# wuwuz/Pacmann

Measured on AMD Instinct MI355X. Metric: private queries/sec + PIR-scan HBM GB/s, SIFT1M d=128 at 1/2/4/8 GPUs, higher is better.
Workload: dtype u64

## Files before the change

### pacmann_amd/csrc/pm_aes.h

```cpp
#pragma once
#include <hip/hip_runtime.h>
#include <stdint.h>

namespace pm {

struct AesTables {
  uint8_t sbox[256];
  uint32_t te0[256];
  constexpr AesTables() : sbox(), te0() {
    for (int x = 0; x < 256; ++x) {
      uint8_t inv = 0;
      if (x) {
        uint8_t r = 1, b = (uint8_t)x;
        int e = 254;
        while (e) {
          if (e & 1) r = gmul(r, b);
          b = gmul(b, b);
          e >>= 1;
        }
        inv = r;
      }
      uint8_t s = inv ^ rotl(inv, 1) ^ rotl(inv, 2) ^ rotl(inv, 3) ^ rotl(inv, 4) ^ 0x63;
      sbox[x] = s;
      uint32_t s2 = gmul(s, 2), s3 = gmul(s, 3);
      te0[x] = s2 | ((uint32_t)s << 8) | ((uint32_t)s << 16) | (s3 << 24);
    }
  }
  static constexpr uint8_t gmul(uint8_t a, uint8_t b) {
    uint8_t p = 0;
    for (int i = 0; i < 8; ++i) {
      if (b & 1) p ^= a;
      bool hi = a & 0x80;
      a = (uint8_t)(a << 1);
      if (hi) a ^= 0x1b;
      b >>= 1;
    }
    return p;
  }
  static constexpr uint8_t rotl(uint8_t v, int n) { return (uint8_t)((v << n) | (v >> (8 - n))); }
};

constexpr int kTeLdsWords = 256 * 64;

static constexpr AesTables kAesTablesHost{};
static __device__ const AesTables g_aes = kAesTablesHost;

__device__ __forceinline__ uint32_t rotl32(uint32_t x, int n) { return (x << n) | (x >> (32 - n)); }
__device__ __forceinline__ uint32_t aes_x3(uint32_t a, uint32_t b, uint32_t c) {
  return __builtin_amdgcn_bitop3_b32(a, b, c, 0x96);
}

__device__ __forceinline__ void aes_lds_init(uint32_t* te, const uint32_t* __restrict__ g_te0) {
  for (int i = threadIdx.x; i < kTeLdsWords; i += blockDim.x) {
    const uint32_t t = g_te0[(i >> 6) & 255];
    te[i] = (i & 32) ? rotl32(t, 16) : t;
  }
}


struct AesLane {
  const uint32_t* te;
  uint32_t lane;
  uint32_t lane2;
  __device__ AesLane(const uint32_t* t, uint32_t tid) : te(t), lane((tid & 31u) << 2), lane2(((tid & 31u) << 2) | 0x80u) {}
  template <int K> __device__ __forceinline__ uint32_t Tk(uint32_t s) const {
    const uint32_t a = __builtin_amdgcn_perm(s, lane, 0x0c0c0000u | ((4u + K) << 8));
    return *reinterpret_cast<const uint32_t*>(reinterpret_cast<const char*>(te) + a);
  }
  template <int K> __device__ __forceinline__ uint32_t T2k(uint32_t s) const {
    const uint32_t a = __builtin_amdgcn_perm(s, lane2, 0x0c0c0000u | ((4u + K) << 8));
    return *reinterpret_cast<const uint32_t*>(reinterpret_cast<const char*>(te) + a);
  }
  template <int K> __device__ __forceinline__ uint32_t Sk(uint32_t s) const { return (Tk<K>(s) >> 8) & 0xffu; }
  __device__ __forceinline__ uint32_t col(uint32_t a, uint32_t b, uint32_t c, uint32_t d, uint32_t k) const {
    return __builtin_amdgcn_bitop3_b32(__builtin_amdgcn_bitop3_b32(Tk<0>(a), T2k<2>(c), k, 0x96),
                                       rotl32(Tk<1>(b) ^ T2k<3>(d), 8), 0u, 0x96);
  }
};

template <int R0 = 1, int R1 = 10>
__device__ __forceinline__ void aes_rounds(const AesLane& A, const uint32_t* __restrict__ rk,
                                           uint32_t& s0, uint32_t& s1, uint32_t& s2, uint32_t& s3) {
#pragma unroll
  for (int r = R0; r < R1; ++r) {
    uint32_t t0 = A.col(s0, s1, s2, s3, rk[4 * r + 0]);
    uint32_t t1 = A.col(s1, s2, s3, s0, rk[4 * r + 1]);
    uint32_t t2 = A.col(s2, s3, s0, s1, rk[4 * r + 2]);
    uint32_t t3 = A.col(s3, s0, s1, s2, rk[4 * r + 3]);
    s0 = t0; s1 = t1; s2 = t2; s3 = t3;
  }
}

__device__ __forceinline__ uint64_t prf64(const AesLane& A, const uint32_t* __restrict__ rk,
                                          uint64_t tag, uint64_t x) {
  const uint64_t b = (tag << 35) + x;
  const uint32_t w0 = (uint32_t)b, w1 = (uint32_t)(b >> 32);
  uint32_t s0 = w0 ^ rk[0], s1 = w1 ^ rk[1], s2 = rk[2], s3 = rk[3];
  aes_rounds(A, rk, s0, s1, s2, s3);
  uint32_t c0 = (A.Sk<0>(s0) | (A.Sk<1>(s1) << 8) | (A.Sk<2>(s2) << 16) | (A.Sk<3>(s3) << 24)) ^ rk[40];
  uint32_t c1 = (A.Sk<0>(s1) | (A.Sk<1>(s2) << 8) | (A.Sk<2>(s3) << 16) | (A.Sk<3>(s0) << 24)) ^ rk[41];
  return ((uint64_t)(c1 ^ w1) << 32) | (uint64_t)(c0 ^ w0);
}

__device__ __forceinline__ uint32_t prf_lo32(const AesLane& A, const uint32_t* __restrict__ rk,
                                             uint64_t tag, uint64_t x) {
  const uint64_t b = (tag << 35) + x;
  const uint32_t w0 = (uint32_t)b, w1 = (uint32_t)(b >> 32);
  uint32_t s0 = w0 ^ rk[0], s1 = w1 ^ rk[1], s2 = rk[2], s3 = rk[3];
  aes_rounds(A, rk, s0, s1, s2, s3);
  uint32_t c0 = (A.Sk<0>(s0) | (A.Sk<1>(s1) << 8) | (A.Sk<2>(s2) << 16) | (A.Sk<3>(s3) << 24)) ^ rk[40];
  return c0 ^ w0;
}

struct R1Uniform { uint32_t u0, u1, u2, u3; };
__device__ __forceinline__ R1Uniform r1_uniform(const AesLane& A, const uint32_t* __restrict__ rk, uint32_t x) {
  const uint32_t s0 = x ^ rk[0], s2 = rk[2], s3 = rk[3];
  return R1Uniform{A.Tk<0>(s0) ^ A.T2k<2>(s2) ^ rotl32(A.T2k<3>(s3), 8) ^ rk[4],
                   A.T2k<2>(s3) ^ rotl32(A.Tk<1>(s2) ^ A.T2k<3>(s0), 8) ^ rk[5],
                   A.Tk<0>(s2) ^ A.T2k<2>(s0) ^ rotl32(A.Tk<1>(s3), 8) ^ rk[6],
                   A.Tk<0>(s3) ^ rotl32(A.Tk<1>(s0) ^ A.T2k<3>(s2), 8) ^ rk[7]};
}
struct R1Lane { uint32_t v0, v1, v2, v3; };
__device__ __forceinline__ R1Lane r1_lane(const AesLane& A, const uint32_t* __restrict__ rk, uint64_t tag) {
  const uint32_t s1 = (uint32_t)(tag << 3) ^ rk[1];
  return R1Lane{rotl32(A.Tk<1>(s1), 8), A.Tk<0>(s1), rotl32(A.T2k<3>(s1), 8), A.T2k<2>(s1)};
}
__device__ __forceinline__ uint32_t prf_lo32_split(const AesLane& A, const uint32_t* __restrict__ rk,
                                                   const R1Uniform& u, const R1Lane& v, uint32_t x) {
  uint32_t s0 = u.u0 ^ v.v0, s1 = u.u1 ^ v.v1, s2 = u.u2 ^ v.v2, s3 = u.u3 ^ v.v3;
  aes_rounds<2>(A, rk, s0, s1, s2, s3);
  const uint32_t c0 = (A.Sk<0>(s0) | (A.Sk<1>(s1) << 8) | (A.Sk<2>(s2) << 16) | (A.Sk<3>(s3) << 24)) ^ rk[40];
  return c0 ^ x;
}

__device__ __forceinline__ uint32_t prf_lo16_split(const AesLane& A, const uint32_t* __restrict__ rk,
                                                   const R1Uniform& u, const R1Lane& v, uint32_t x) {
  uint32_t s0 = u.u0 ^ v.v0, s1 = u.u1 ^ v.v1, s2 = u.u2 ^ v.v2, s3 = u.u3 ^ v.v3;
  aes_rounds<2, 9>(A, rk, s0, s1, s2, s3);
  const uint32_t t0 = A.col(s0, s1, s2, s3, rk[36]);
  const uint32_t t1 = A.col(s1, s2, s3, s0, rk[37]);
  return ((A.Sk<0>(t0) | (A.Sk<1>(t1) << 8)) ^ rk[40] ^ x) & 0xffffu;
}
struct R2Hint { uint32_t k0, k1, k2, k3; };
__device__ __forceinline__ R2Hint r2_hint(const AesLane& A, const uint32_t* __restrict__ rk, const R1Uniform& u,
                                          const R1Lane& v) {
  const uint32_t s1 = u.u1 ^ v.v1, s2 = u.u2 ^ v.v2, s3 = u.u3 ^ v.v3;
  return R2Hint{A.T2k<2>(s2) ^ rk[8] ^ rotl32(A.Tk<1>(s1) ^ A.T2k<3>(s3), 8),
                A.Tk<0>(s1) ^ A.T2k<2>(s3) ^ rk[9] ^ rotl32(A.Tk<1>(s2), 8),
                A.Tk<0>(s2) ^ rk[10] ^ rotl32(A.Tk<1>(s3) ^ A.T2k<3>(s1), 8),
                A.Tk<0>(s3) ^ A.T2k<2>(s1) ^ rk[11] ^ rotl32(A.T2k<3>(s2), 8)};
}
__device__ __forceinline__ uint32_t prf_lo16_r2(const AesLane& A, const uint32_t* __restrict__ rk, uint32_t u0,
                                                const R1Lane& v, const R2Hint& k, uint32_t x) {
  const uint32_t s = u0 ^ v.v0;
  uint32_t s0 = A.Tk<0>(s) ^ k.k0, s1 = rotl32(A.T2k<3>(s), 8) ^ k.k1;
  uint32_t s2 = A.T2k<2>(s) ^ k.k2, s3 = rotl32(A.Tk<1>(s), 8) ^ k.k3;
  aes_rounds<3, 9>(A, rk, s0, s1, s2, s3);
  const uint32_t t0 = A.col(s0, s1, s2, s3, rk[36]);
  const uint32_t t1 = A.col(s1, s2, s3, s0, rk[37]);
  return ((A.Sk<0>(t0) | (A.Sk<1>(t1) << 8)) ^ rk[40] ^ x) & 0xffffu;
}
}
```

### pacmann_amd/csrc/pm_kernels.hip

```cpp
#include <atomic>
#include "pm_aes.h"
#include "pm_aes_bs.h"
#include "pm_internal.h"

namespace pm {
#ifndef PM_PREP_NT
#define PM_PREP_NT 0
#endif


__device__ __forceinline__ uint32_t xor3(uint32_t a, uint32_t b, uint32_t c) {
  return __builtin_amdgcn_bitop3_b32(a, b, c, 0x96);
}
__device__ __forceinline__ uint4 xor4(uint4 a, uint4 b) {
  return make_uint4(a.x ^ b.x, a.y ^ b.y, a.z ^ b.z, a.w ^ b.w);
}

#ifndef PM_OFFS_CHUNKS
#define PM_OFFS_CHUNKS 8
#endif
constexpr int kOffsChunksPerBlock = PM_OFFS_CHUNKS;
constexpr int kOffsBlock = 1024;

#ifndef PM_OFFS_TILES
#define PM_OFFS_TILES 1
#endif
constexpr int kOffsTiles = PM_OFFS_TILES;
__global__ void __launch_bounds__(kOffsBlock, 1) k_prep_offsets(const PmPart* __restrict__ parts) {
  __shared__ uint32_t te[kTeLdsWords];
  __shared__ R1Uniform r1u[kOffsTiles][kOffsChunksPerBlock];
  const PmPart& P = parts[blockIdx.z];
  const uint32_t H = P.H, SS = P.SS;
  const uint32_t cb = blockIdx.y * kOffsChunksPerBlock * kOffsTiles;
  if (blockIdx.x * kOffsBlock >= H || cb >= SS) return;
  aes_lds_init(te, g_aes.te0);
  __syncthreads();
  const AesLane A(te, threadIdx.x);
  const uint32_t cend = min(SS, cb + kOffsChunksPerBlock * kOffsTiles);
  if (threadIdx.x < cend - cb)
    r1u[threadIdx.x / kOffsChunksPerBlock][threadIdx.x % kOffsChunksPerBlock] = r1_uniform(A, P.rk, cb + threadIdx.x);
  __syncthreads();
  const uint32_t h = blockIdx.x * kOffsBlock + threadIdx.x;
  if (h >= H) return;
  const uint32_t mask = P.CS - 1;
  const uint32_t own = h >= P.PH ? (h - P.PH) / P.Qpc : 0xffffffffu;
  uint16_t* o = P.tab;
  const R1Lane r1v = r1_lane(A, P.rk, h);
  const bool r2 = SS <= 256;
  const R2Hint r2k = r2 ? r2_hint(A, P.rk, r1u[0][0], r1v) : R2Hint{0, 0, 0, 0};
  static_assert(kOffsChunksPerBlock == 8, "one 16-B tabT tile of 8 chunks per thread");
  for (int tl = 0; tl < kOffsTiles; ++tl) {
    const uint32_t c0 = cb + tl * kOffsChunksPerBlock;
    if (c0 >= SS) break;
    const uint32_t c1 = min(SS, c0 + kOffsChunksPerBlock);
    uint16_t tile[8];
#pragma unroll
    for (int j = 0; j < 8; ++j) tile[j] = kSkip;
    auto put = [&](uint32_t c, uint32_t prf) {
      uint16_t v = (uint16_t)(prf & mask);
      v = (c == own) ? kSkip : v;
      if (o) o[(uint64_t)c * H + h] = v;
      tile[c - c0] = v;
      if (h < P.PH) P.cur[cur_index(P.PH, P.curk, c, h)] = v;
    };
    for (uint32_t c = c0; c < c1; ++c)
      put(c, r2 ? prf_lo16_r2(A, P.rk, r1u[tl][c - c0].u0, r1v, r2k, c) : prf_lo16_split(A, P.rk, r1u[tl][c - c0], r1v, c));
    uint4 t4;
    t4.x = tile[0] | ((uint32_t)tile[1] << 16); t4.y = tile[2] | ((uint32_t)tile[3] << 16);
    t4.z = tile[4] | ((uint32_t)tile[5] << 16); t4.w = tile[6] | ((uint32_t)tile[7] << 16);
    if (PM_PREP_NT) {
      typedef uint32_t u32x4 __attribute__((ext_vector_type(4)));
      __builtin_nontemporal_store(u32x4{t4.x, t4.y, t4.z, t4.w}, reinterpret_cast<u32x4*>(P.tabT + tabT_index(H, h, c0)));
    } else {
      *reinterpret_cast<uint4*>(P.tabT + tabT_index(H, h, c0)) = t4;
    }
  }
}

constexpr int kBsThreads = 256;
#ifndef PM_BS_WAVES
#define PM_BS_WAVES 2
#endif
__global__ void __launch_bounds__(kBsThreads, PM_BS_WAVES) k_prep_offsets_bs(const PmPart* __restrict__ parts) {
  __shared__ uint32_t bs_te0[256];
  __shared__ uint32_t bs_kx[32];
  __shared__ uint32_t bs_wv[32][4];
  __shared__ __attribute__((aligned(16))) uint32_t bs_wp[128];
  __shared__ __attribute__((aligned(16))) uint32_t bs_stash[16 * kBsThreads];
  const PmPart& P = parts[blockIdx.y];
  const uint32_t H = P.H, SS = P.SS, PH = P.PH;
  const uint32_t nm = (H + 31) / 32, ng = (SS + 7) / 8;
  if (blockIdx.x * kBsThreads >= nm * ng) return;
  bs_te0[threadIdx.x] = g_aes.te0[threadIdx.x];
  __syncthreads();
  bs_setup_a(bs_te0, P.rk, bs_kx, bs_wv);
  __syncthreads();
  bs_setup_b(bs_wv, bs_wp);
  __syncthreads();
  const uint32_t task = blockIdx.x * kBsThreads + threadIdx.x;
  if (task >= nm * ng) return;
  const uint32_t m = task % nm, g = task / nm, h0 = 32 * m;
  const uint32_t nb = P.log2CS, Qpc = P.Qpc;
  const uint32_t keep = nb >= 16 ? 0xffffu : (1u << nb) - 1u;
  auto lowmask = [](int n) { return n <= 0 ? 0u : n >= 32 ? ~0u : (1u << n) - 1u; };
  uint4* stash = reinterpret_cast<uint4*>(bs_stash) + threadIdx.x;
#pragma unroll 1
  for (uint32_t q = 0; q < 8; ++q) {
    const uint32_t cc = 8 * g + q, c = cc & ~1u;
    uint32_t T[32];
    if (c < SS) {
      uint32_t o[16];
      bs_prf16(bs_te0, P.rk, bs_kx, bs_wp, m, cc, o);
      const int lo = (int)(PH + cc * Qpc) - (int)h0, hi = lo + (int)Qpc;
      const uint32_t own = lowmask(hi) & ~lowmask(lo);
#pragma unroll
      for (int b = 0; b < 16; ++b) o[b] = (((keep >> b) & 1u) ? o[b] : 0u) | own;
      if ((q & 1) == 0) {
#pragma unroll
        for (int i = 0; i < 4; ++i) stash[i * kBsThreads] = make_uint4(o[4 * i], o[4 * i + 1], o[4 * i + 2], o[4 * i + 3]);
        continue;
      }
#pragma unroll
      for (int i = 0; i < 4; ++i) {
        const uint4 v = stash[i * kBsThreads];
        T[4 * i] = v.x; T[4 * i + 1] = v.y; T[4 * i + 2] = v.z; T[4 * i + 3] = v.w;
      }
#pragma unroll
      for (int b = 0; b < 16; ++b) T[16 + b] = o[b];
      bs_transpose32(T);
    } else {
      if ((q & 1) == 0) continue;
#pragma unroll
      for (int j = 0; j < 32; ++j) T[j] = 0xffffffffu;
    }
    uint32_t* tt = reinterpret_cast<uint32_t*>(P.tabT + tabT_index(H, h0, c));
    if (h0 + 32 <= H) {
#pragma unroll
      for (int j = 0; j < 32; ++j) tt[4 * j] = T[j];
    } else {
#pragma unroll
      for (int j = 0; j < 32; ++j)
        if (h0 + j < H) tt[4 * j] = T[j];
    }
    if (c >= SS) continue;
#pragma unroll
    for (int jb = 0; jb < 4; ++jb) {
      const uint32_t hb = h0 + 8 * jb;
      uint4 wlo, whi;
      wlo.x = __builtin_amdgcn_perm(T[8 * jb + 1], T[8 * jb + 0], 0x05040100u);
      wlo.y = __builtin_amdgcn_perm(T[8 * jb + 3], T[8 * jb + 2], 0x05040100u);
      wlo.z = __builtin_amdgcn_perm(T[8 * jb + 5], T[8 * jb + 4], 0x05040100u);
      wlo.w = __builtin_amdgcn_perm(T[8 * jb + 7], T[8 * jb + 6], 0x05040100u);
      whi.x = __builtin_amdgcn_perm(T[8 * jb + 1], T[8 * jb + 0], 0x07060302u);
      whi.y = __builtin_amdgcn_perm(T[8 * jb + 3], T[8 * jb + 2], 0x07060302u);
      whi.z = __builtin_amdgcn_perm(T[8 * jb + 5], T[8 * jb + 4], 0x07060302u);
      whi.w = __builtin_amdgcn_perm(T[8 * jb + 7], T[8 * jb + 6], 0x07060302u);
      if (hb < PH) {
        *reinterpret_cast<uint4*>(P.cur + cur_index(PH, P.curk, c, hb)) = wlo;
        *reinterpret_cast<uint4*>(P.cur + cur_index(PH, P.curk, c + 1, hb)) = whi;
      }
      if (P.tab && hb < H) {
        *reinterpret_cast<uint4*>(P.tab + (uint64_t)c * H + hb) = wlo;
        *reinterpret_cast<uint4*>(P.tab + (uint64_t)(c + 1) * H + hb) = whi;
      }
    }
  }
}

#ifndef PM_FOLD_NT
#define PM_FOLD_NT 1
#endif
template <int W>
__global__ void __launch_bounds__(kBlock) k_prep_fold(const PmPart* __restrict__ parts,
                                                      const uint64_t* __restrict__ db, uint32_t E) {
  const PmPart& P = parts[blockIdx.y];
  const uint32_t EX = E & ~3u, NSEG = EX / W;
  const uint64_t e = (uint64_t)blockIdx.x * kBlock + threadIdx.x;
  const uint32_t H = P.H;
  if (NSEG == 0) {
    if (e < (uint64_t)H * E) P.parity[e] = 0;
    return;
  }
  const uint32_t h = (uint32_t)(e / NSEG), seg = (uint32_t)(e % NSEG);
  if (h >= H) return;
  const uint64_t* base = db + (P.row0 * E) + (uint64_t)seg * W;
  const uint32_t CS = P.CS, SS = P.SS;
  const uint64_t N = P.N;
  uint64_t a0 = 0, a1 = 0;
  uint32_t c = 0;
  for (; c + 4 <= SS; c += 4) {
    const uint64_t t4 = *reinterpret_cast<const uint64_t*>(P.tabT + tabT_index(H, h, c));
    uint16_t v[4];
#pragma unroll
    for (int u = 0; u < 4; ++u) v[u] = (uint16_t)(t4 >> (16 * u));
#pragma unroll
    for (int u = 0; u < 4; ++u) {
      const uint64_t r = (uint64_t)(c + u) * CS + v[u];
      if (v[u] != kSkip && r < N) {
        const uint64_t* p = base + r * E;
        if (W == 2) {
          typedef uint32_t u32x4 __attribute__((ext_vector_type(4)));
          const u32x4 x = PM_FOLD_NT ? __builtin_nontemporal_load(reinterpret_cast<const u32x4*>(p))
                                     : *reinterpret_cast<const u32x4*>(p);
          a0 ^= ((uint64_t)x.y << 32) | x.x;
          a1 ^= ((uint64_t)x.w << 32) | x.z;
        } else {
          a0 ^= PM_FOLD_NT ? __builtin_nontemporal_load(p) : *p;
        }
      }
    }
  }
  for (; c < SS; ++c) {
    uint16_t v = P.tabT[tabT_index(H, h, c)];
    const uint64_t r = (uint64_t)c * CS + v;
    if (v != kSkip && r < N) {
      const uint64_t* p = base + r * E;
      a0 ^= p[0];
      if (W == 2) a1 ^= p[1];
    }
  }
  uint64_t* dst = P.parity + (uint64_t)h * E + (uint64_t)seg * W;
  dst[0] = a0;
  if (W == 2) dst[1] = a1;
  if (seg == 0)
    for (uint32_t w = EX; w < E; ++w) P.parity[(uint64_t)h * E + w] = 0;
}

constexpr int kFoldThreads = 1024, kFoldHPT = 7;
// ... 565 lines not shown
          if (r >= P.N) continue;
          const uint64_t* p = base + r * rw + (uint64_t)seg * W;
          if (W == 2) {
            const uint4 x = *reinterpret_cast<const uint4*>(p);
            x0[u] = ((uint64_t)x.y << 32) | x.x;
            x1[u] = ((uint64_t)x.w << 32) | x.z;
          } else {
            x0[u] = *p;
          }
        }
#pragma unroll
        for (uint32_t u = 0; u < kSrvFlight; ++u) { a0 ^= x0[u]; a1 ^= x1[u]; }
      }
    }
    red[threadIdx.x * 2] = a0;
    red[threadIdx.x * 2 + 1] = a1;
    __syncthreads();
    if (threadIdx.x < nseg) {
      uint64_t x0 = 0, x1 = 0;
      for (uint32_t k = 0; k < nsl; ++k) {
        x0 ^= red[(k * nseg + threadIdx.x) * 2];
        x1 ^= red[(k * nseg + threadIdx.x) * 2 + 1];
      }
      if (PK && seg < cseg) {
        const uint32_t v[4] = {(uint32_t)x0, (uint32_t)(x0 >> 32), (uint32_t)x1, (uint32_t)(x1 >> 32)};
#pragma unroll
        for (uint32_t k = 0; k < 4; ++k)
          out[4 * seg + k] = ((uint64_t)(v[k] & 0xffff0000u) << 32) | (uint64_t)(uint32_t)(v[k] << 16);
      } else if (PK) {
        out[4 * cseg + 2 * (seg - cseg)] = x0;
        out[4 * cseg + 2 * (seg - cseg) + 1] = x1;
      } else {
        out[(uint64_t)seg * W] = x0;
        if (W == 2) out[(uint64_t)seg * W + 1] = x1;
      }
    }
    __syncthreads();
  }
  for (uint32_t w = (E & ~3u) + threadIdx.x; w < E; w += kBlock) out[w] = 0;
}

__global__ void __launch_bounds__(kBlock) k_l2_rows(const float* __restrict__ rows,
                                                    uint64_t stride, uint64_t nrows,
                                                    const uint32_t* __restrict__ ids,
                                                    const float* __restrict__ q, uint32_t dim,
                                                    float* __restrict__ out, uint64_t seglen) {
  const uint64_t g = ((uint64_t)blockIdx.x * kBlock + threadIdx.x) >> 3;
  const uint32_t k = threadIdx.x & 7;
  const bool live = g < nrows;
  const float* r = rows + (live ? (ids ? (uint64_t)ids[g] : g) : 0) * stride;
  if (seglen && live) q += (g / seglen) * dim;
  const uint32_t dimS = dim & ~7u;
  float acc = 0.0f;
  if (live)
    for (uint32_t t = k; t < dimS; t += 8) {
      const float d = __fsub_rn(r[t], q[t]);
      acc = __fadd_rn(acc, __fmul_rn(d, d));
    }
  acc = __fadd_rn(acc, __shfl_xor(acc, 1));
  acc = __fadd_rn(acc, __shfl_xor(acc, 2));
  acc = __fadd_rn(acc, __shfl_xor(acc, 4));
  if (live && k == 0) {
    float d = dimS ? acc : 0.0f;
    for (uint32_t i = dimS; i < dim; ++i) {
      const float t = __fsub_rn(r[i], q[i]);
      d = __fadd_rn(d, __fmul_rn(t, t));
    }
    out[g] = d;
  }
}

__global__ void __launch_bounds__(kBlock) k_ip_rows(const uint32_t* __restrict__ rows, uint64_t nrows,
                                                    const uint32_t* __restrict__ q, uint32_t dim,
                                                    uint32_t* __restrict__ per_row,
                                                    uint32_t* __restrict__ sum) {
  const uint64_t g = ((uint64_t)blockIdx.x * kBlock + threadIdx.x) >> 4;
  const uint32_t l = threadIdx.x & 15;
  uint32_t acc = 0;
  if (g < nrows) {
    const uint32_t* r = rows + g * dim;
    for (uint32_t j = l; j < dim; j += 16) acc += r[j] * q[j];
  }
#pragma unroll
  for (int m = 1; m < 16; m <<= 1) acc += __shfl_xor(acc, m);
  if (g < nrows && l == 0 && per_row) per_row[g] = acc;
  uint32_t w = (l == 0 && g < nrows) ? acc : 0;
#pragma unroll
  for (int m = 16; m < 64; m <<= 1) w += __shfl_xor(w, m);
  if ((threadIdx.x & 63) == 0) atomicAdd(sum, w);
}

__global__ void __launch_bounds__(kBlock) k_ip_scan(const uint4* __restrict__ rows, uint64_t n4,
                                                    const uint32_t* __restrict__ q, uint32_t dim,
                                                    uint32_t* __restrict__ sum) {
  __shared__ uint32_t qs[4096];
  for (uint32_t j = threadIdx.x; j < dim; j += kBlock) qs[j] = q[j];
  __syncthreads();
  uint32_t acc = 0;
  const uint64_t stride = (uint64_t)gridDim.x * kBlock;
  const uint32_t dim4 = dim / 4;
  typedef unsigned int u32x4 __attribute__((ext_vector_type(4)));
  const u32x4* r4 = reinterpret_cast<const u32x4*>(rows);
  uint64_t f = (uint64_t)blockIdx.x * kBlock + threadIdx.x;
  if (stride % dim4 == 0) {
    const uint32_t j = (uint32_t)(f % dim4) * 4;
    const uint32_t q0 = qs[j], q1 = qs[j + 1], q2 = qs[j + 2], q3 = qs[j + 3];
    constexpr int kU = 8;
    for (; f + (kU - 1) * stride < n4; f += kU * stride) {
      u32x4 t[kU];
#pragma unroll
      for (int u = 0; u < kU; ++u) t[u] = __builtin_nontemporal_load(r4 + f + u * stride);
#pragma unroll
      for (int u = 0; u < kU; ++u) acc += t[u].x * q0 + t[u].y * q1 + t[u].z * q2 + t[u].w * q3;
    }
    for (; f < n4; f += stride) {
      const u32x4 t = __builtin_nontemporal_load(r4 + f);
      acc += t.x * q0 + t.y * q1 + t.z * q2 + t.w * q3;
    }
  } else {
    for (; f < n4; f += stride) {
      const u32x4 t = __builtin_nontemporal_load(r4 + f);
      const uint32_t j = (uint32_t)(f % dim4) * 4;
      acc += t.x * qs[j] + t.y * qs[j + 1] + t.z * qs[j + 2] + t.w * qs[j + 3];
    }
  }
#pragma unroll
  for (int m = 1; m < 64; m <<= 1) acc += __shfl_xor(acc, m);
  if ((threadIdx.x & 63) == 0) atomicAdd(sum, acc);
}

__global__ void __launch_bounds__(kBlock) k_ip_fill(uint4* __restrict__ rows, uint64_t n4, uint32_t dim,
                                                    uint64_t r0) {
  const uint64_t stride = (uint64_t)gridDim.x * kBlock;
  for (uint64_t f = (uint64_t)blockIdx.x * kBlock + threadIdx.x; f < n4; f += stride) {
    const uint64_t e = f * 4;
    const uint32_t i = (uint32_t)(r0 + e / dim), j = (uint32_t)(e % dim);
    rows[f] = make_uint4(i + j, i + j + 1, i + j + 2, i + j + 3);
  }
}

__global__ void __launch_bounds__(kBlock) k_db_synth(uint64_t* __restrict__ dst, uint64_t r0, uint64_t nw,
                                                     uint32_t E, uint64_t k) {
  const uint64_t stride = (uint64_t)gridDim.x * kBlock, x0 = r0 * E;
  for (uint64_t f = (uint64_t)blockIdx.x * kBlock + threadIdx.x; f < nw; f += stride)
    __builtin_nontemporal_store(sm64(k ^ (x0 + f)), dst + f);
}

__global__ void __launch_bounds__(kBlock) k_prf_batch(const uint32_t* __restrict__ rk,
                                                      const uint64_t* __restrict__ tags,
                                                      const uint64_t* __restrict__ xs, uint64_t n,
                                                      uint64_t* __restrict__ out) {
  __shared__ uint32_t te[kTeLdsWords];
  __shared__ uint32_t srk[44];
  aes_lds_init(te, g_aes.te0);
  if (threadIdx.x < 44) srk[threadIdx.x] = rk[threadIdx.x];
  __syncthreads();
  const AesLane A(te, threadIdx.x);
  for (uint64_t i = (uint64_t)blockIdx.x * kBlock + threadIdx.x; i < n; i += (uint64_t)gridDim.x * kBlock)
    out[i] = prf64(A, srk, tags[i], xs[i]);
}

__global__ void __launch_bounds__(kBlock) k_gather_rows(const uint64_t* const* __restrict__ src, uint32_t E,
                                                         uint64_t* __restrict__ out) {
  const uint64_t i = blockIdx.x;
  const uint64_t* r = src[i];
  uint64_t* o = out + i * (E + 1);
  for (uint32_t w = threadIdx.x; w < E; w += kBlock) o[w] = r ? r[w] : 0;
  if (threadIdx.x == 0) o[E] = r ? 1 : 0;
}

}

namespace pmk {
static inline unsigned cdiv(uint64_t a, uint64_t b) { return (unsigned)((a + b - 1) / b); }

void prep_init(hipStream_t st, const PmPart* d, int np, uint32_t maxH, uint32_t maxRepl, uint32_t,
               bool) {
  const uint32_t n = maxH > maxRepl ? maxH : maxRepl;
  hipLaunchKernelGGL(k_prep_init, dim3(cdiv(n, kBlock), np), dim3(kBlock), 0, st, d);
}
void prep_offsets_tt(hipStream_t st, const PmPart* d, int np, uint32_t maxH, uint32_t maxSS) {
  hipLaunchKernelGGL(k_prep_offsets, dim3(cdiv(maxH, kOffsBlock), cdiv(maxSS, kOffsChunksPerBlock * kOffsTiles), np),
                     dim3(kOffsBlock), 0, st, d);
}
void prep_offsets_bs(hipStream_t st, const PmPart* d, int np, uint32_t maxH, uint32_t maxSS) {
  hipLaunchKernelGGL(k_prep_offsets_bs, dim3(cdiv((uint64_t)cdiv(maxH, 32) * cdiv(maxSS, 8), kBsThreads), np),
                     dim3(kBsThreads), 0, st, d);
}
static std::atomic<int> g_aes_bs{-1};
void set_aes_bs(int v) { g_aes_bs.store(v < 0 ? -1 : (v ? 1 : 0)); }
bool prep_offsets_bitsliced() {
  static const bool env = [] { const char* e = getenv("PM_AES_BS"); return e && e[0] == '1'; }();
  const int v = g_aes_bs.load();
  return v < 0 ? env : v == 1;
}
void prep_offsets(hipStream_t st, const PmPart* d, int np, uint32_t maxH, uint32_t maxSS) {
  if (prep_offsets_bitsliced()) prep_offsets_bs(st, d, np, maxH, maxSS);
  else prep_offsets_tt(st, d, np, maxH, maxSS);
}
static std::atomic<int> g_fold_rot{-1};
void set_fold_rot(int v) { g_fold_rot.store(v < 0 ? -1 : (v ? 1 : 0)); }
static bool fold_rot_shape(uint32_t minCS, uint32_t maxCS, uint32_t E) {
  return minCS == maxCS && (maxCS == 512 || maxCS == 1024) && E % 2 == 0 && E >= 4;
}
bool fold_image_ok(uint32_t minCS, uint32_t maxCS, uint32_t E) {
  static const bool env = [] { const char* e = getenv("PM_FOLD_ROT"); return !e || e[0] != '0'; }();
  const int v = g_fold_rot.load();
  return (v < 0 ? env : v == 1) && fold_rot_shape(minCS, maxCS, E);
}
static uint32_t fold_blk_sw(uint32_t maxCS) {
  auto fits = [&](uint32_t sw) {
    return 2ull * (maxCS + 1) * sw * 8 <= 150u * 1024 &&
           (uint64_t)maxCS * (sw / 2) <= (uint64_t)kFoldMaxItems * kFoldThreads;
  };
  uint32_t sw = 8;
  while (sw > 2 && !fits(sw)) sw /= 2;
  return fits(sw) ? sw : 0;
}
int fold_form(uint32_t minCS, uint32_t maxCS, uint32_t E, bool have_img, uint32_t npk) {
  if ((E & ~3u) == 0) return FOLD_GATHER;
  if (have_img && fold_rot_shape(minCS, maxCS, E))
    return maxCS == 512 ? (npk ? FOLD_ROT512P : FOLD_ROT512) : FOLD_ROT1024;
  if (minCS == maxCS && (maxCS == 512 || maxCS == 1024 || maxCS == 2048) && E % 2 == 0) return FOLD_PIPE;
  if (E % 2 || !fold_blk_sw(maxCS)) return FOLD_GATHER;
  return FOLD_BLK;
}
bool fold_needs_tab(uint32_t minCS, uint32_t maxCS, uint32_t E, bool have_img) {
  const int form = fold_form(minCS, maxCS, E, have_img);
  return form == FOLD_PIPE || form == FOLD_BLK;
}
static std::atomic<int> g_fold_pack{-1};
void set_fold_pack(int v) { g_fold_pack.store(v < 0 ? -1 : (v ? 1 : 0)); }
uint32_t fold_pack_slices(uint32_t minCS, uint32_t maxCS, uint32_t E, uint32_t dim) {
  static const bool env = [] { const char* e = getenv("PM_FOLD_PACK"); return !e || e[0] != '0'; }();
  const int v = g_fold_pack.load();
  if (!(v < 0 ? env : v == 1) || fold_form(minCS, maxCS, E, true) != FOLD_ROT512) return 0;
  return fold_pack_shape(E, dim);
}
uint32_t fold_pack_shape(uint32_t E, uint32_t dim) {
  return dim && dim % 16 == 0 && dim / 8 <= E / 4 ? dim / 16 : 0;
}
static std::atomic<int> g_answer_pack{-1};
void set_answer_pack(int v) { g_answer_pack.store(v < 0 ? -1 : (v ? 1 : 0)); }
uint32_t answer_pack_shape(uint32_t E, uint32_t dim) {
  if (!dim || E % 4 || E > 256 || dim % 8 || dim >= 2 * E) return 0;
  const uint32_t stride = 2 * dim + 4 * (2 * E - dim);
  return stride % 16 ? 0 : stride / 16;
}
uint32_t answer_pack_segs(uint32_t E, uint32_t dim) {
  static const bool env = [] { const char* e = getenv("PM_ANSWER_PACK"); return !e || e[0] != '0'; }();
  const int v = g_answer_pack.load();
  return (v < 0 ? env : v == 1) ? answer_pack_shape(E, dim) : 0;
}
void answer_pack_image(hipStream_t st, uint64_t* img, const uint64_t* rows, uint64_t nrows, uint32_t E, uint32_t dim) {
  const uint32_t nseg = answer_pack_shape(E, dim);
  const uint64_t nitems = nrows * nseg;
  unsigned grid = cdiv(nitems, kBlock);
  if (grid > 256 * 32) grid = 256 * 32;
  if (grid) hipLaunchKernelGGL(k_answer_pack_image, dim3(grid), dim3(kBlock), 0, st, (uint4*)img, rows, nitems, E, nseg, dim / 8);
}
bool coord_low_zero(hipStream_t st, const uint64_t* rows, uint64_t nrows, uint32_t E, uint32_t dim, uint32_t* flag) {
  if (hipMemsetAsync(flag, 0, 4, st) != hipSuccess) return false;
  unsigned grid = cdiv(nrows * (dim / 4), kBlock);
  if (grid > 256 * 32) grid = 256 * 32;
  if (grid) hipLaunchKernelGGL(k_coord_low_or, dim3(grid), dim3(kBlock), 0, st, rows, nrows, E, dim, flag);
  uint32_t h = 1;
  if (hipMemcpyAsync(&h, flag, 4, hipMemcpyDeviceToHost, st) != hipSuccess || hipStreamSynchronize(st) != hipSuccess)
    return false;
  return h == 0;
}
uint64_t fold_image_words(uint32_t SS, uint32_t E, uint32_t CS, uint32_t npk) {
  return (uint64_t)(E / 4 - npk) * (SS / rot_nch(CS)) * (kRotBufBytes / 8);
}
void fold_image(hipStream_t st, uint64_t* img, const uint64_t* rows, uint64_t N, uint32_t SS, uint32_t E, uint32_t CS,
                uint32_t npk) {
  const uint64_t nitems = fold_image_words(SS, E, CS, npk) / 2;
  unsigned grid = cdiv(nitems, kBlock);
  if (grid > 256 * 32) grid = 256 * 32;
  hipLaunchKernelGGL(k_fold_image, dim3(grid), dim3(kBlock), 0, st, (uint4*)img, rows, N, SS / rot_nch(CS), E, nitems,
                     CS, npk);
}
void fold_image_map(uint32_t CS, uint32_t SS, uint32_t npk, uint64_t x0, uint64_t n, uint64_t* row, uint32_t* word,
                    uint8_t* packed) {
  for (uint64_t i = 0; i < n; ++i) {
    const FoldImageSrc s = fold_image_src(x0 + i, SS / rot_nch(CS), CS, npk);
    row[i] = s.row; word[i] = s.word; packed[i] = s.packed;
  }
}
int prep_fold(hipStream_t st, const PmPart* d, int np, uint32_t maxH, const uint64_t* db, uint32_t E,
              uint32_t minCS, uint32_t maxCS, const uint64_t* zero16, uint32_t clients, bool have_img,
               uint32_t minH, uint32_t npk) {
  const int form = fold_form(minCS, maxCS, E, have_img, npk);
  const uint32_t EX = E & ~3u;
  if (EX == 0) {
    hipLaunchKernelGGL(k_prep_fold<2>, dim3(cdiv((uint64_t)maxH * E, kBlock), np), dim3(kBlock), 0,
                       st, d, db, E);
    return form;
  }
  const uint32_t ng = cdiv(maxH, (uint64_t)kFoldThreads * kFoldHPT);
  const uint32_t ngb = cdiv(maxH, (uint64_t)kFoldThreads * kFoldHPTBlk);
  auto launch = [&](uint32_t sw, uint32_t w0, uint32_t nsl) {
    const size_t lds = 2ull * (maxCS + 1) * sw * 8;
    const dim3 grid(ngb, nsl, np), blk(kFoldThreads);
    if (sw == 8) hipLaunchKernelGGL(k_prep_fold_blk<8>, grid, blk, lds, st, d, db, zero16, E, w0);
    else if (sw == 4) hipLaunchKernelGGL(k_prep_fold_blk<4>, grid, blk, lds, st, d, db, zero16, E, w0);
    else hipLaunchKernelGGL(k_prep_fold_blk<2>, grid, blk, lds, st, d, db, zero16, E, w0);
  };
// ... 123 lines not shown
```

Measured before the change: 28560.

## Specialize offset-prep kernel by round-2 and tab flags, pair PRF outputs

Rewrites k_prep_offsets into a templated tile routine specialized on whether the round-2 shortcut applies and whether the tab output exists, removing per-element branches. PRF results are computed two chunks at a time and packed with perm/bitop3 into 32-bit words. Per-element cur_index math is replaced by incremental row pointers, and the skip entry is patched once after the loop. The LDS AES table init is fully unrolled with a compile-time thread count. This adds template code size and register pressure in exchange for fewer ALU ops and branches in the hint preprocessing path.

New measurement: 29020, median of 6. 1.6% higher.

```diff
diff --git a/pacmann_amd/csrc/pm_aes.h b/pacmann_amd/csrc/pm_aes.h
--- a/pacmann_amd/csrc/pm_aes.h
+++ b/pacmann_amd/csrc/pm_aes.h
@@ -50,10 +50,16 @@
   return __builtin_amdgcn_bitop3_b32(a, b, c, 0x96);
 }
 
+template <int NT>
 __device__ __forceinline__ void aes_lds_init(uint32_t* te, const uint32_t* __restrict__ g_te0) {
-  for (int i = threadIdx.x; i < kTeLdsWords; i += blockDim.x) {
-    const uint32_t t = g_te0[(i >> 6) & 255];
-    te[i] = (i & 32) ? rotl32(t, 16) : t;
+  static_assert(NT % 64 == 0 && kTeLdsWords % NT == 0, "whole 64-word entry rows per pass");
+  const uint32_t rot = (threadIdx.x & 32u) ? 16u : 0u;
+  const uint32_t* src = g_te0 + (threadIdx.x >> 6);
+  uint32_t* dst = te + threadIdx.x;
+#pragma unroll
+  for (int k = 0; k < kTeLdsWords / NT; ++k) {
+    const uint32_t t = src[NT / 64 * k];
+    dst[NT * k] = __builtin_amdgcn_alignbit(t, t, rot);
   }
 }
 
@@ -133,13 +139,22 @@
   return c0 ^ x;
 }
 
-__device__ __forceinline__ uint32_t prf_lo16_split(const AesLane& A, const uint32_t* __restrict__ rk,
-                                                   const R1Uniform& u, const R1Lane& v, uint32_t x) {
+struct Lo16Words { uint32_t w0, w1; };
+__device__ __forceinline__ Lo16Words lo16_tail(const AesLane& A, const uint32_t* __restrict__ rk, uint32_t s0,
+                                               uint32_t s1, uint32_t s2, uint32_t s3) {
+  const uint32_t t0 = A.col(s0, s1, s2, s3, rk[36]);
+  const uint32_t t1 = A.col(s1, s2, s3, s0, rk[37]);
+  return Lo16Words{A.Tk<0>(t0), A.Tk<1>(t1)};
+}
+__device__ __forceinline__ uint32_t lo16_pair(const Lo16Words& a, const Lo16Words& b, uint32_t x2) {
+  return __builtin_amdgcn_bitop3_b32(__builtin_amdgcn_perm(a.w1, a.w0, 0x0c0c0501u),
+                                     __builtin_amdgcn_perm(b.w1, b.w0, 0x05010c0cu), x2, 0x56);
+}
+__device__ __forceinline__ Lo16Words prf_lo16_split(const AesLane& A, const uint32_t* __restrict__ rk,
+                                                    const R1Uniform& u, const R1Lane& v) {
   uint32_t s0 = u.u0 ^ v.v0, s1 = u.u1 ^ v.v1, s2 = u.u2 ^ v.v2, s3 = u.u3 ^ v.v3;
   aes_rounds<2, 9>(A, rk, s0, s1, s2, s3);
-  const uint32_t t0 = A.col(s0, s1, s2, s3, rk[36]);
-  const uint32_t t1 = A.col(s1, s2, s3, s0, rk[37]);
-  return ((A.Sk<0>(t0) | (A.Sk<1>(t1) << 8)) ^ rk[40] ^ x) & 0xffffu;
+  return lo16_tail(A, rk, s0, s1, s2, s3);
 }
 struct R2Hint { uint32_t k0, k1, k2, k3; };
 __device__ __forceinline__ R2Hint r2_hint(const AesLane& A, const uint32_t* __restrict__ rk, const R1Uniform& u,
@@ -150,14 +165,12 @@
                 A.Tk<0>(s2) ^ rk[10] ^ rotl32(A.Tk<1>(s3) ^ A.T2k<3>(s1), 8),
                 A.Tk<0>(s3) ^ A.T2k<2>(s1) ^ rk[11] ^ rotl32(A.T2k<3>(s2), 8)};
 }
-__device__ __forceinline__ uint32_t prf_lo16_r2(const AesLane& A, const uint32_t* __restrict__ rk, uint32_t u0,
-                                                const R1Lane& v, const R2Hint& k, uint32_t x) {
+__device__ __forceinline__ Lo16Words prf_lo16_r2(const AesLane& A, const uint32_t* __restrict__ rk, uint32_t u0,
+                                                 const R1Lane& v, const R2Hint& k) {
   const uint32_t s = u0 ^ v.v0;
   uint32_t s0 = A.Tk<0>(s) ^ k.k0, s1 = rotl32(A.T2k<3>(s), 8) ^ k.k1;
   uint32_t s2 = A.T2k<2>(s) ^ k.k2, s3 = rotl32(A.Tk<1>(s), 8) ^ k.k3;
   aes_rounds<3, 9>(A, rk, s0, s1, s2, s3);
-  const uint32_t t0 = A.col(s0, s1, s2, s3, rk[36]);
-  const uint32_t t1 = A.col(s1, s2, s3, s0, rk[37]);
-  return ((A.Sk<0>(t0) | (A.Sk<1>(t1) << 8)) ^ rk[40] ^ x) & 0xffffu;
+  return lo16_tail(A, rk, s0, s1, s2, s3);
 }
 }
diff --git a/pacmann_amd/csrc/pm_kernels.hip b/pacmann_amd/csrc/pm_kernels.hip
--- a/pacmann_amd/csrc/pm_kernels.hip
+++ b/pacmann_amd/csrc/pm_kernels.hip
@@ -26,54 +26,108 @@
 #define PM_OFFS_TILES 1
 #endif
 constexpr int kOffsTiles = PM_OFFS_TILES;
+
+__device__ __forceinline__ void store16_row(PM_G uint16_t* row, uint32_t lane_bytes, uint32_t v) {
+  *reinterpret_cast<PM_G uint16_t*>(reinterpret_cast<PM_G char*>(row) + lane_bytes) = (uint16_t)v;
+}
+
+template <bool R2, bool TAB>
+__device__ __forceinline__ void prep_offsets_tiles(const PmPart& P, const AesLane& A,
+                                                   const R1Uniform (&r1u)[kOffsTiles][kOffsChunksPerBlock],
+                                                   const uint32_t (&r1u0)[kOffsTiles][kOffsChunksPerBlock],
+                                                   uint32_t cb, uint32_t h) {
+  const uint32_t H = P.H, SS = P.SS, PH = P.PH, K = P.curk;
+  const uint32_t m = P.CS - 1, m2 = m | (m << 16);
+  const uint32_t k2 = (P.rk[40] & 0xffffu) * 0x10001u;
+  const bool prim = h < PH;
+  const uint32_t own = prim ? 0xffffffffu : (h - PH) / P.Qpc;
+  const uint32_t lcur = cur_row_off(K, h) * 2, ltab = h * 2;
+  const uint64_t cur_group = (uint64_t)cur_blocks(PH) * K * 8;
+  const R1Lane r1v = r1_lane(A, P.rk, h);
+  R2Hint r2k{0, 0, 0, 0};
+  if (R2) r2k = r2_hint(A, P.rk, r1u[0][0], r1v);
+  for (int tl = 0; tl < kOffsTiles; ++tl) {
+    const uint32_t c0 = cb + tl * kOffsChunksPerBlock;
+    if (c0 >= SS) break;
+    const uint32_t c1 = min(SS, c0 + kOffsChunksPerBlock);
+    const uint32_t cq = K == 2 ? c0 >> 1 : K == 1 ? c0 : c0 / K;
+    uint32_t cr = c0 - cq * K;
+    uint64_t crow = cq * cur_group + cr * 8;
+    auto next_cur = [&] {
+      if (++cr == K) { cr = 0; crow += cur_group - (K - 1) * 8; }
+      else crow += 8;
+    };
+    uint64_t trow = (uint64_t)c0 * H;
+    uint32_t w[4] = {0xffffffffu, 0xffffffffu, 0xffffffffu, 0xffffffffu};
+    uint32_t u0[kOffsChunksPerBlock];
+#pragma unroll
+    for (int i = 0; i < kOffsChunksPerBlock; ++i) u0[i] = R2 ? r1u0[tl][i] : 0u;
+#pragma unroll
+    for (int p = 0; p < 4; ++p) {
+      const uint32_t c = c0 + 2 * p;
+      if (c >= c1) break;
+      const Lo16Words a = R2 ? prf_lo16_r2(A, P.rk, u0[2 * p], r1v, r2k) : prf_lo16_split(A, P.rk, r1u[tl][2 * p], r1v);
+      const Lo16Words b = R2 ? prf_lo16_r2(A, P.rk, u0[2 * p + 1], r1v, r2k) : prf_lo16_split(A, P.rk, r1u[tl][2 * p + 1], r1v);
+      const uint32_t kx = k2 ^ (c | ((c + 1) << 16));
+      const uint32_t v = lo16_pair(a, b, kx) & m2;
+      w[p] = v;
+      if (TAB) {
+        store16_row(P.tab + trow, ltab, v);
+        store16_row(P.tab + trow + H, ltab, v >> 16);
+        trow += 2 * (uint64_t)H;
+      }
+      const uint64_t crow_a = crow;
+      next_cur();
+      const uint64_t crow_b = crow;
+      next_cur();
+      if (prim) {
+        store16_row(P.cur + crow_a, lcur, v);
+        store16_row(P.cur + crow_b, lcur, v >> 16);
+      }
+    }
+    const uint32_t j = own - c0;
+    if (j < c1 - c0) {
+      const uint32_t half = (j & 1) ? 0xffff0000u : 0x0000ffffu;
+#pragma unroll
+      for (uint32_t p = 0; p < 4; ++p) w[p] |= (j >> 1) == p ? half : 0u;
+      if (TAB) P.tab[(uint64_t)own * H + h] = kSkip;
+    }
+    if (PM_PREP_NT) {
+      typedef uint32_t u32x4 __attribute__((ext_vector_type(4)));
+      __builtin_nontemporal_store(u32x4{w[0], w[1], w[2], w[3]}, reinterpret_cast<u32x4*>(P.tabT + tabT_index(H, h, c0)));
+    } else {
+      *reinterpret_cast<uint4*>(P.tabT + tabT_index(H, h, c0)) = make_uint4(w[0], w[1], w[2], w[3]);
+    }
+  }
+}
+
 __global__ void __launch_bounds__(kOffsBlock, 1) k_prep_offsets(const PmPart* __restrict__ parts) {
   __shared__ uint32_t te[kTeLdsWords];
   __shared__ R1Uniform r1u[kOffsTiles][kOffsChunksPerBlock];
+  __shared__ __attribute__((aligned(16))) uint32_t r1u0[kOffsTiles][kOffsChunksPerBlock];
   const PmPart& P = parts[blockIdx.z];
   const uint32_t H = P.H, SS = P.SS;
   const uint32_t cb = blockIdx.y * kOffsChunksPerBlock * kOffsTiles;
   if (blockIdx.x * kOffsBlock >= H || cb >= SS) return;
-  aes_lds_init(te, g_aes.te0);
+  aes_lds_init<kOffsBlock>(te, g_aes.te0);
   __syncthreads();
   const AesLane A(te, threadIdx.x);
   const uint32_t cend = min(SS, cb + kOffsChunksPerBlock * kOffsTiles);
-  if (threadIdx.x < cend - cb)
-    r1u[threadIdx.x / kOffsChunksPerBlock][threadIdx.x % kOffsChunksPerBlock] = r1_uniform(A, P.rk, cb + threadIdx.x);
+  if (threadIdx.x < cend - cb) {
+    const R1Uniform u = r1_uniform(A, P.rk, cb + threadIdx.x);
+    r1u[threadIdx.x / kOffsChunksPerBlock][threadIdx.x % kOffsChunksPerBlock] = u;
+    r1u0[threadIdx.x / kOffsChunksPerBlock][threadIdx.x % kOffsChunksPerBlock] = u.u0;
+  }
   __syncthreads();
   const uint32_t h = blockIdx.x * kOffsBlock + threadIdx.x;
   if (h >= H) return;
-  const uint32_t mask = P.CS - 1;
-  const uint32_t own = h >= P.PH ? (h - P.PH) / P.Qpc : 0xffffffffu;
-  uint16_t* o = P.tab;
-  const R1Lane r1v = r1_lane(A, P.rk, h);
-  const bool r2 = SS <= 256;
-  const R2Hint r2k = r2 ? r2_hint(A, P.rk, r1u[0][0], r1v) : R2Hint{0, 0, 0, 0};
   static_assert(kOffsChunksPerBlock == 8, "one 16-B tabT tile of 8 chunks per thread");
-  for (int tl = 0; tl < kOffsTiles; ++tl) {
-    const uint32_t c0 = cb + tl * kOffsChunksPerBlock;
-    if (c0 >= SS) break;
-    const uint32_t c1 = min(SS, c0 + kOffsChunksPerBlock);
-    uint16_t tile[8];
-#pragma unroll
-    for (int j = 0; j < 8; ++j) tile[j] = kSkip;
-    auto put = [&](uint32_t c, uint32_t prf) {
-      uint16_t v = (uint16_t)(prf & mask);
-      v = (c == own) ? kSkip : v;
-      if (o) o[(uint64_t)c * H + h] = v;
-      tile[c - c0] = v;
-      if (h < P.PH) P.cur[cur_index(P.PH, P.curk, c, h)] = v;
-    };
-    for (uint32_t c = c0; c < c1; ++c)
-      put(c, r2 ? prf_lo16_r2(A, P.rk, r1u[tl][c - c0].u0, r1v, r2k, c) : prf_lo16_split(A, P.rk, r1u[tl][c - c0], r1v, c));
-    uint4 t4;
-    t4.x = tile[0] | ((uint32_t)tile[1] << 16); t4.y = tile[2] | ((uint32_t)tile[3] << 16);
-    t4.z = tile[4] | ((uint32_t)tile[5] << 16); t4.w = tile[6] | ((uint32_t)tile[7] << 16);
-    if (PM_PREP_NT) {
-      typedef uint32_t u32x4 __attribute__((ext_vector_type(4)));
-      __builtin_nontemporal_store(u32x4{t4.x, t4.y, t4.z, t4.w}, reinterpret_cast<u32x4*>(P.tabT + tabT_index(H, h, c0)));
-    } else {
-      *reinterpret_cast<uint4*>(P.tabT + tabT_index(H, h, c0)) = t4;
-    }
+  if (SS <= 256) {
+    if (P.tab) prep_offsets_tiles<true, true>(P, A, r1u, r1u0, cb, h);
+    else prep_offsets_tiles<true, false>(P, A, r1u, r1u0, cb, h);
+  } else {
+    if (P.tab) prep_offsets_tiles<false, true>(P, A, r1u, r1u0, cb, h);
+    else prep_offsets_tiles<false, false>(P, A, r1u, r1u0, cb, h);
   }
 }
 
@@ -945,7 +999,7 @@
                                                       uint64_t* __restrict__ out) {
   __shared__ uint32_t te[kTeLdsWords];
   __shared__ uint32_t srk[44];
-  aes_lds_init(te, g_aes.te0);
+  aes_lds_init<kBlock>(te, g_aes.te0);
   if (threadIdx.x < 44) srk[threadIdx.x] = rk[threadIdx.x];
   __syncthreads();
   const AesLane A(te, threadIdx.x);
```
